# tau-dev/SdfBox

Hardware: AMD Instinct MI355X
Metric: Mray/s (primary rays; frame W*H / time per frame) (higher is better)
Workload: dtype f32

## Files before the change

sdfbox_amd/csrc/raymarch_device.h:

```cpp
#pragma once
#include <hip/hip_runtime.h>
#include <stdint.h>

namespace sdfhip {

typedef uint4 NodeRec;


struct FrameInfo {
    float h0x, h0y, h0z, h1x, h1y, h1z, h2x, h2y, h2z;
    float posx, posy, posz, margin;
    float screen_w, screen_h, limit;
    float lightx, lighty, lightz;
    float fov, k_strength;
    float margin2;
    float half_aspect;
};
constexpr int MAX_BATCH = 8;
constexpr int MAX_BAND_LIST = 512;
constexpr int INLINE_BAND_LIST = 64;

struct TopCell { uint32_t level, v0, v1; int32_t children; };
struct GridRef {
    const TopCell *top; const TopCell *fine; int level; int fine_bits; int fine_order;
#ifdef SDFHIP_EXPERIMENTS
    const uint32_t *d4 = nullptr; const uint4 *recs = nullptr;
    uint32_t *touch_top = nullptr, *touch_fine = nullptr; uint32_t touch_top_words = 0, touch_fine_words = 0;
#endif
};
#ifdef SDFHIP_EXPERIMENTS
__device__ __forceinline__ void touch_line(uint32_t *bits, uint32_t words, uint32_t cell)
// ... 33 lines not shown
    uint32_t n_band_list;
    uint16_t band_list[INLINE_BAND_LIST];
    const uint16_t *band_ptr;
    uint32_t tiles_x, tiles_y, n_tiles;
    uint32_t n_frames;
    FrameInfo frames[MAX_BATCH];
    unsigned long long *counters;
    uint32_t *queue;
#ifdef SDFHIP_EXPERIMENTS
    uint32_t tile_order;
#endif
    uint32_t out_mode;
    uint32_t sparse_cap;
    uint32_t sparse_base;
    uint32_t sky8;
    uint32_t out_host;
    uint32_t pt_spp, pt_bounces, pt_seed;
    float pt_albedo;
    float4 *hit_a;
    int4 *hit_b;
    uint4 *hit_c;
    float4 *hit_d;
    uint32_t *hit_ctl;
    uint32_t hit_cap, hit_set;
    uint32_t hit_min;
    float4 *pt_q[2];
    uint32_t *pt_ctl;
    uint32_t pt_cap, pt_level;
    float *pt_e;
    float *pt_t;
// ... 147 lines not shown
        ax = ay = az = 0; level = 0;
        children = (int32_t)root.y; v0 = root.z; v1 = root.w;
    }
    __device__ __forceinline__ Cell cell() const
    {
        Cell k;
        const float q = 1.0f / 4096.0f;
        k.lx = (float)ax * q; k.ly = (float)ay * q; k.lz = (float)az * q;
        k.scale = __int_as_float((127 - level) << 23);
        k.inv = __int_as_float((127 + level) << 23);
        k.v0 = v0; k.v1 = v1;
        return k;
    }
};

__device__ __forceinline__ int32_t axis_a(float p, float &u, float &f)
{
    u = p * 4096.0f;
    f = floorf(u);
    return (int32_t)__builtin_amdgcn_fmed3f(f, -2.0f, 4097.0f);
}
__device__ __forceinline__ int bitlen(uint32_t x) { return 32 - __clz((int)x); }

template <bool ON_GRID>
__device__ __forceinline__ uint32_t find_s(CursorS &c, const NodeRec *__restrict__ nodes,
                                           const TopCell *__restrict__ top, const int TG,
                                           int32_t *__restrict__ stack, uint32_t stride,
                                           int32_t Ax, int32_t Ay, int32_t Az, bool gx, bool gy, bool gz)
{
    const int32_t Bx = Ax - ((ON_GRID && gx) ? 1 : 0);
    const int32_t By = Ay - ((ON_GRID && gy) ? 1 : 0);
    const int32_t Bz = Az - ((ON_GRID && gz) ? 1 : 0);
    const int s = LM - c.level;
// ... 43 lines not shown
            c.v1 = r.w;
            asm volatile("" : "+v"(c.v0), "+v"(c.v1));
            c.level++;
            reads++; c.loads++;
        }
        const int32_t keep = ~((1 << (LM - c.level)) - 1);
        c.ax = Dx & keep; c.ay = Dy & keep; c.az = Dz & keep;
    } else if (k > 0) {
        const int32_t keep = ~((1 << (LM - c.level)) - 1);
        c.ax &= keep; c.ay &= keep; c.az &= keep;
    }
    return reads;
}

constexpr uint32_t FLAT_BIT = 0x80000000u;
template <bool EXACT, bool SPLIT, bool ORDERED = false>
struct CursorFT {
    typedef Scaled Pos;
    static constexpr int32_t ROOT_MARK = 0x40000000;
    int32_t ax, ay, az;
    uint32_t s;
    uint32_t v0, v1;
    uint32_t sh;
    uint32_t loads;

    __device__ __forceinline__ void reset(const NodeRec &root)
    {
        ax = ay = az = ROOT_MARK; s = (uint32_t)LM; v0 = root.z; v1 = root.w; sh = 0;
    }
    __device__ __forceinline__ int4 pack() const
    {
        const bool fresh = ax == ROOT_MARK;
        return make_int4(fresh ? ax : (int32_t)((uint32_t)ax << sh), fresh ? ay : (int32_t)((uint32_t)ay << sh), fresh ? az : (int32_t)((uint32_t)az << sh), (int32_t)s);
// ... 7 lines not shown
    __device__ __forceinline__ static uint32_t units_shift(int full_level) { return EXACT ? 0u : (uint32_t)(LM - full_level); }
    __device__ __forceinline__ Cell cell() const
    {
        Cell k;
        const float q = 1.0f / 4096.0f;
        const bool fresh = ax == ROOT_MARK;
        const int32_t keep = (int32_t)(0xFFFFFFFFu << (s & 31u));
        const int32_t x = (int32_t)((uint32_t)ax << sh) & keep, y = (int32_t)((uint32_t)ay << sh) & keep, z = (int32_t)((uint32_t)az << sh) & keep;
        k.lx = fresh ? 0.0f : (float)x * q; k.ly = fresh ? 0.0f : (float)y * q; k.lz = fresh ? 0.0f : (float)z * q;
        const uint32_t sc = s & 15u;
        k.scale = __uint_as_float((127u - LM + sc) << 23);
        k.inv = __uint_as_float((127u + LM - sc) << 23);
        k.v0 = v0; k.v1 = (s & FLAT_BIT) ? v0 : v1;
        return k;
    }
};

template <bool EXACT, bool SPLIT, bool ORDERED>
__device__ __forceinline__ int load_cell(CursorFT<EXACT, SPLIT, ORDERED> &c, const GridRef &g, int32_t Dx, int32_t Dy, int32_t Dz)
{
    const int TG = g.level, sh = LM - TG;
    const uint32_t ti = top_index((uint32_t)Dx >> sh, (uint32_t)Dy >> sh, (uint32_t)Dz >> sh, TG);
    uint4 e = reinterpret_cast<const uint4 *>(g.top)[ti];
    c.loads++;
#ifdef SDFHIP_EXPERIMENTS
    if (EXACT && g.touch_top) touch_line(g.touch_top, g.touch_top_words, ti);
#endif
    if (SPLIT) {
        asm volatile("" : "+v"(e.y), "+v"(e.z), "+v"(e.w));
        if (e.x == 15u) {
// ... 2 lines not shown
            const uint32_t m = (1u << FB) - 1u;
            const uint32_t local = fine_cell_index(((uint32_t)Dx >> sh2) & m, ((uint32_t)Dy >> sh2) & m, ((uint32_t)Dz >> sh2) & m, FB, ORDERED ? g.fine_order : 0);
#ifdef SDFHIP_EXPERIMENTS
            if (EXACT && g.touch_fine) touch_line(g.touch_fine, g.touch_fine_words, e.w + local);
#endif
            e = reinterpret_cast<const uint4 *>(g.fine)[e.w + local];
        }
    }
    c.s = e.x;
    c.v0 = e.y;
    c.v1 = e.z;
    c.ax = Dx; c.ay = Dy; c.az = Dz;
    return (int)(e.x & 15u);
}

template <bool SPLIT, bool ORDERED>
__device__ __forceinline__ void load_cell_units(CursorFT<false, SPLIT, ORDERED> &c, const GridRef &g, int32_t Dx, int32_t Dy, int32_t Dz)
{
    uint4 e;
    c.loads++;
    if (!SPLIT) {
        e = reinterpret_cast<const uint4 *>(g.top)[top_index((uint32_t)Dx, (uint32_t)Dy, (uint32_t)Dz, g.level)];
    } else {
        const int FB = g.fine_bits;
        e = reinterpret_cast<const uint4 *>(g.top)[top_index((uint32_t)Dx >> FB, (uint32_t)Dy >> FB, (uint32_t)Dz >> FB, g.level)];
        asm volatile("" : "+v"(e.y), "+v"(e.z), "+v"(e.w));
        if (e.x == 15u) {
            c.loads++;
            const uint32_t m = (1u << FB) - 1u;
            const uint32_t local = fine_cell_index((uint32_t)Dx & m, (uint32_t)Dy & m, (uint32_t)Dz & m, FB, ORDERED ? g.fine_order : 0);
            e = reinterpret_cast<const uint4 *>(g.fine)[e.w + local];
            asm volatile("" : "+v"(e.y), "+v"(e.z), "+v"(e.w));
// ... 40 lines not shown
    }
    uint32_t reads = 1u;
    if (moved) {
        Dx = min(max(Dx, 0), 4095); Dy = min(max(Dy, 0), 4095); Dz = min(max(Dz, 0), 4095);
        const int ns = load_cell(c, g, Dx, Dy, Dz);
        reads = 1u + (uint32_t)k + (uint32_t)((LM - ns) - (level - k));
    }
    return reads;
}
__device__ __forceinline__ int32_t cvt_floor(float u)
{
    int32_t a;
    asm("v_cvt_flr_i32_f32_e32 %0, %1" : "=v"(a) : "v"(u));
    return a;
}
template <bool SPLIT, bool FRESH, bool ORDERED>
__device__ __forceinline__ uint32_t find_units(CursorFT<false, SPLIT, ORDERED> &c, const GridRef &g, float px, float py, float pz, Scaled &u)
{
    const int F = g.level + (SPLIT ? g.fine_bits : 0), sh = LM - F;
    const float unit = __uint_as_float((uint32_t)(127 + F) << 23), top = unit - 1.0f;
    u.x = px * unit; u.y = py * unit; u.z = pz * unit;
    const float fx = __builtin_amdgcn_fractf(u.x), fy = __builtin_amdgcn_fractf(u.y), fz = __builtin_amdgcn_fractf(u.z);
    const float fm = __builtin_fminf(__builtin_fminf(fx, fy), fz);
    int32_t Dx, Dy, Dz;
    if (FRESH || __builtin_expect(__ballot(fm == 0.0f) == 0ull, 1)) {
        Dx = cvt_floor(__builtin_amdgcn_fmed3f(u.x, 0.0f, top)); Dy = cvt_floor(__builtin_amdgcn_fmed3f(u.y, 0.0f, top));
        Dz = cvt_floor(__builtin_amdgcn_fmed3f(u.z, 0.0f, top));
    } else {
        float tx, ty, tz, qx, qy, qz;
        Dx = axis_a(px, tx, qx); Dy = axis_a(py, ty, qy); Dz = axis_a(pz, tz, qz);
        const int4 k = c.pack();
        bool moved;
        on_face_choice(k.x, k.y, k.z, (int)(c.s & 15u), Dx, Dy, Dz, tx == qx, ty == qy, tz == qz, moved);
        Dx = min(max(Dx, 0), 4095) >> sh; Dy = min(max(Dy, 0), 4095) >> sh; Dz = min(max(Dz, 0), 4095) >> sh;
    }
    c.sh = (uint32_t)sh;
    load_cell_units(c, g, Dx, Dy, Dz);
    return 0;
}
template <bool SPLIT, bool ORDERED>
__device__ __forceinline__ uint32_t find(CursorFT<false, SPLIT, ORDERED> &c, const NodeRec *__restrict__, const GridRef &g,
                                         uint32_t, int32_t *__restrict__, uint32_t, float px, float py, float pz,
                                         Scaled &u)
{
    return find_units<SPLIT, false, ORDERED>(c, g, px, py, pz, u);
}
template <class CursorT, class Pos>
__device__ __forceinline__ uint32_t find_fresh(CursorT &c, const NodeRec *__restrict__ nodes, const GridRef &g, uint32_t n,
                                               int32_t *__restrict__ stack, uint32_t stride, float px, float py, float pz, Pos &u)
{
    return find(c, nodes, g, n, stack, stride, px, py, pz, u);
}
template <bool SPLIT, bool ORDERED>
__device__ __forceinline__ uint32_t find_fresh(CursorFT<false, SPLIT, ORDERED> &c, const NodeRec *__restrict__, const GridRef &g,
                                               uint32_t, int32_t *__restrict__, uint32_t, float px, float py, float pz,
                                               Scaled &u)
{
    return find_units<SPLIT, true, ORDERED>(c, g, px, py, pz, u);
}
template <bool SPLIT, bool ORDERED>
__device__ __forceinline__ uint32_t find(CursorFT<true, SPLIT, ORDERED> &c, const NodeRec *__restrict__, const GridRef &g,
                                         uint32_t, int32_t *__restrict__, uint32_t, float px, float py, float pz,
                                         Scaled &u)
{
    float fx, fy, fz;
    const int32_t Ax = axis_a(px, u.x, fx), Ay = axis_a(py, u.y, fy), Az = axis_a(pz, u.z, fz);
    const bool gx = u.x == fx, gy = u.y == fy, gz = u.z == fz;
    return find_full(c, g, Ax, Ay, Az, gx, gy, gz, __ballot(gx || gy || gz) != 0ull);
}
template <bool EXACT, bool SPLIT, bool ORDERED>
__device__ __forceinline__ float sample_after_find(const CursorFT<EXACT, SPLIT, ORDERED> &c, const Scaled &u, float, float, float)
{
    if (c.s & FLAT_BIT) return __uint_as_float(c.v1);
    const float scale = __uint_as_float((c.s + (uint32_t)(127 - LM)) << 23);
    const uint32_t k = c.s - c.sh;
    const float inv = __uint_as_float((127u - k) << 23);
    const int32_t keep = (int32_t)(0xFFFFFFFFu << (k & 31u));
    float dx = sat((u.x - (float)(c.ax & keep)) * inv);
    float dy = sat((u.y - (float)(c.ay & keep)) * inv);
    float dz = sat((u.z - (float)(c.az & keep)) * inv);
    Texels t = decode(c.v0, c.v1);
    float loadL = bilerp(t.v[0], t.v[1], t.v[2], t.v[3], dx, dy);
    float loadH = bilerp(t.v[4], t.v[5], t.v[6], t.v[7], dx, dy);
    return (lerp(loadL, loadH, dz) - 0.25f) * scale * 2.0f;
}
__device__ __forceinline__ uint32_t flat_cell_distance_bits(uint32_t byte, uint32_t s)
{
    const float scale = __uint_as_float((s + (uint32_t)(127 - LM)) << 23);
    return __float_as_uint((unorm8((float)byte) - 0.25f) * scale * 2.0f);
}
// ... 114 lines not shown
```

sdfbox_amd/csrc/raymarch_kernels.h:

```cpp
#pragma once
#include "raymarch_device.h"

namespace sdfhip {

constexpr int MAX_STACK = LM;
#ifndef COMPACT_WAVES_PER_SIMD
#define COMPACT_WAVES_PER_SIMD 8
#endif
#ifndef PATH_WAVES_PER_SIMD
#define PATH_WAVES_PER_SIMD 7
#endif
#ifndef PLAIN_WAVES_PER_SIMD
#define PLAIN_WAVES_PER_SIMD 8
#endif

enum { CUR_GENERIC = 0, CUR_STACK = 1, CUR_STACK_FULL = 2, CUR_STACK_SPLIT = 3, CUR_DENSE4 = 4 };
template <int CUR, bool COUNT> struct CursorOf { typedef CursorG type; };
template <bool COUNT> struct CursorOf<CUR_STACK, COUNT> { typedef CursorS type; };
template <bool COUNT> struct CursorOf<CUR_STACK_FULL, COUNT> { typedef CursorFT<COUNT, false> type; };
template <bool COUNT> struct CursorOf<CUR_STACK_SPLIT, COUNT> { typedef CursorFT<COUNT, true> type; };
__device__ __forceinline__ GridRef grid_of(const RenderParams &P, const TopCell *top = nullptr)
{
#ifdef SDFHIP_EXPERIMENTS
    return GridRef{top ? top : P.top, P.fine, P.top_level, P.fine_bits, P.fine_order, P.d4, P.recs,
                   P.touch_top, P.touch_fine, P.touch_top_words, P.touch_fine_words};
#else
    return GridRef{top ? top : P.top, P.fine, P.top_level, P.fine_bits, P.fine_order};
#endif
}
template <class CursorT>
__device__ __forceinline__ Cell cell_of(const CursorT &c, const RenderParams &) { return c.cell(); }
#ifdef SDFHIP_EXPERIMENTS
template <> struct CursorOf<CUR_DENSE4, false> { typedef CursorFF type; };
__device__ __forceinline__ Cell cell_of(const CursorFF &c, const RenderParams &P) { return cell_of(c, grid_of(P), P.nodes); }
#endif
template <int CUR, bool COUNT> struct ScatterCursorOf { typedef typename CursorOf<CUR, COUNT>::type type; };
template <bool COUNT> struct ScatterCursorOf<CUR_STACK_SPLIT, COUNT> { typedef CursorFT<COUNT, true, true> type; };

enum { PH_PRIMARY = 0, PH_SHADOW = 1, PH_SHADE = 2, PH_IDLE = 3, PH_DONE = 4 };

struct RayState {
    float px, py, pz;
    float dx, dy, dz;
    float prox, angle, dist;
    int n, base, phase;
};
// ... 2 lines not shown
{
    if (!P.n_band_list && P.band_first == 0u && P.band_stride == 1u) return yl;
    const uint32_t band = P.band_shift < 32u ? yl >> P.band_shift : yl / P.band_rows, within = yl - band * P.band_rows;
    if (P.n_band_list) {
        if (band >= P.n_band_list) return 0xFFFFFFFFu;
        const uint32_t b = P.n_band_list <= (uint32_t)INLINE_BAND_LIST ? P.band_list[band] : P.band_ptr[band];
        return b * P.band_rows + within;
    }
    return (P.band_first + band * P.band_stride) * P.band_rows + within;
}

template <class CursorT>
__device__ __forceinline__ void start_pixel(const FrameInfo &I, const NodeRec &root, uint32_t x,
                                            uint32_t y, RayState &r, CursorT &c)
{
    r.px = I.posx; r.py = I.posy; r.pz = I.posz;
    ray(I, x, y, r.dx, r.dy, r.dz);
    r.prox = 1.0f;
    r.angle = 0.0f; r.dist = 0.0f;
    r.n = 0; r.base = 0; r.phase = PH_PRIMARY;
    c.reset(root);
}


__device__ __forceinline__ uint32_t to_unorm8(float c) { return (uint32_t)(sat(c) * 255.0f + 0.5f); }
__device__ __forceinline__ uint32_t gamma8(float c) { return to_unorm8(powf(c, 1.0f / 2.2f)); }
__device__ __forceinline__ uint32_t alpha8(float steps) { return steps >= 1.0f ? 0xFF000000u : 0u; }
__device__ __forceinline__ uint32_t heat8(float steps)
{
    uint32_t q = to_unorm8(steps / 140.0f);
    return q | (q << 8) | (q << 16);
}
__device__ __forceinline__ uint32_t display8(const float4 &v, uint32_t mode)
// ... 117 lines not shown
        if (s == 2) return true;
        if (shade(I, r, c, dst)) return true;
    }
    return check_shadow(I, r, c, dst);
}

template <class CursorT, bool FRESH = false>
__device__ __forceinline__ uint32_t march_step(const RenderParams &P, const FrameInfo &I, RayState &r, CursorT &c,
                                               int32_t *stack, uint32_t stride, const TopCell *top = nullptr)
{
    typename CursorT::Pos u;
    const GridRef g = grid_of(P, top);
    uint32_t reads = FRESH ? find_fresh(c, P.nodes, g, P.n_nodes, stack, stride, r.px, r.py, r.pz, u)
                           : find(c, P.nodes, g, P.n_nodes, stack, stride, r.px, r.py, r.pz, u);
    r.prox = sample_after_find(c, u, r.px, r.py, r.pz);
    float step = r.phase ? r.prox + I.margin : r.prox;
    r.px = __builtin_fmaf(r.dx, step, r.px);
    r.py = __builtin_fmaf(r.dy, step, r.py);
    r.pz = __builtin_fmaf(r.dz, step, r.pz);
    r.n++;
    return reads;
}

#ifndef SDFHIP_EXPERIMENTS
struct StepClasses {};
template <class CursorT>
__device__ __forceinline__ void classify_step(StepClasses &, const CursorT &, const RenderParams &, float, float, float) {}
__device__ __forceinline__ void flush_classes(const RenderParams &, StepClasses &) {}
#else
struct StepClasses { unsigned long long n[6] = {0, 0, 0, 0, 0, 0}; };
template <class CursorT>
// ... 210 lines not shown
{
    const uint32_t xcd = (bid + frame * (P.tiles_y & 7u)) & 7u, j = bid >> 3;
    const uint32_t r = j / P.tiles_x, cx = j - r * P.tiles_x;
    const uint32_t row = r * 8 + xcd;
    return row < P.tiles_y ? row * P.tiles_x + cx : 0xFFFFFFFFu;
}
__device__ __forceinline__ uint32_t *hit_count(const RenderParams &P, uint32_t set, uint32_t f, uint32_t q)
{
    return P.hit_ctl + (((size_t)set * MAX_BATCH + f) * HIT_QUEUES + q) * 32u;
}

template <bool COUNT, class CursorT>
__device__ __forceinline__ bool shadow_march(const RenderParams &P, const FrameInfo &I, RayState &r, CursorT &c,
                                             unsigned long long &cn, unsigned long long &cs, StepClasses *classes = nullptr)
{
    auto header = [&]() { return r.n < 40 && r.prox > -I.margin; };
    auto at_light = [&]() {
        const float lo = __builtin_fminf(__builtin_fminf(r.px, r.py), r.pz), hi = __builtin_fmaxf(__builtin_fmaxf(r.px, r.py), r.pz);
        return r.prox > r.dist || lo < 0.0f || hi > 1.0f;
    };
    for (;;) {
        bool go = ((int)header() & (int)!at_light()) != 0;
        if (go && r.prox < I.margin) {
            float gx, gy, gz;
            gradient(cell_of(c, P), r.px, r.py, r.pz, gx, gy, gz);
            go = !(dot3(gx, gy, gz, r.dx, r.dy, r.dz) < 0.0f);
        }
        if (!go) break;
        const float qx = r.px, qy = r.py, qz = r.pz;
        uint32_t reads = march_step(P, I, r, c, nullptr, 0);
        if (COUNT) { cn += reads; cs += 1; if (classes) classify_step(*classes, c, P, qx, qy, qz); }
    }
    asm volatile("" : "+v"(r.prox), "+v"(r.n));
    return header() && at_light();
}

template <int CUR, bool COUNT, int MODE, bool QUEUE = false>
__global__ __launch_bounds__(64, PLAIN_WAVES_PER_SIMD) void k_march(RenderParams P)
{
    typedef typename CursorOf<CUR, COUNT>::type CursorT;
    const uint32_t f = blockIdx.y;
    FrameInfo I = P.frames[f];
    asm volatile("" : "+s"(I.margin2), "+s"(I.limit));
    {
        const uint32_t a0 = P.width, a1 = P.height, a2 = P.nrows_out, a3 = P.tiles_x, a4 = P.tiles_y, a5 = P.n_band_list, a6 = P.band_first,
                       a7 = P.band_stride, a8 = P.n_tiles;
        const int32_t b0 = P.top_level, b1 = P.fine_bits;
        const void *p0 = P.nodes, *p1 = P.top, *p2 = P.fine, *p3 = P.out, *p4 = P.tile_perm, *p5 = P.tile_cost;
        asm volatile("" :: "s"(a0), "s"(a1), "s"(a2), "s"(a3), "s"(a4), "s"(a5), "s"(a6), "s"(a7), "s"(a8), "s"(b0), "s"(b1),
                     "s"(p0), "s"(p1), "s"(p2), "s"(p3), "s"(p4), "s"(p5));
    }
    uint32_t tile, tx, ty;
    if (P.tile_perm) {
        const uint32_t wg = blockIdx.z * gridDim.x + blockIdx.x;
        const uint32_t e = P.tile_perm[(wg & 7u) * P.perm_per_label + (wg >> 3)];
        tx = e & 0xFFFFu; ty = e >> 16;
        if (ty >= P.tiles_y || tx >= P.tiles_x) return;
        tile = ty * P.tiles_x + tx;
// ... 4 lines not shown
        tile = ty * P.tiles_x + tx;
    }
    const uint32_t lane = threadIdx.x;
    const uint32_t x = tx * 8 + (lane & 7u), yl = ty * 8 + (lane >> 3);
    unsigned long long cn = 0, cs = 0, ct = 0;
    StepClasses classes;
    SparseLane wire_px{0.0f, 0u};
    bool live = x < P.width && yl < P.nrows_out;
    uint32_t y = 0;
    if (live) { y = global_row(P, yl); live = y < P.height; }
    RayState r;
    CursorT c;
    c.loads = 0;
    const NodeRec root = P.nodes[0];
    start_pixel(I, root, live ? x : 0u, live ? y : 0u, r, c);
    auto marching = [&]() { return (r.prox > I.margin2 || r.prox < 0.0f) && r.n < 100; };
    if (live) {
        auto go_on = [&]() { return ((int)marching() & (int)!(dot3(r.px, r.py, r.pz, r.px, r.py, r.pz) > I.limit)) != 0; };
        if (go_on()) {
            float qx = r.px, qy = r.py, qz = r.pz;
            uint32_t reads = march_step<CursorT, true>(P, I, r, c, nullptr, 0);
            if (COUNT) { cn += reads; cs += 1; classify_step(classes, c, P, qx, qy, qz); }
            while (go_on()) {
                if (COUNT) { qx = r.px; qy = r.py; qz = r.pz; }
                reads = march_step(P, I, r, c, nullptr, 0);
                if (COUNT) { cn += reads; cs += 1; classify_step(classes, c, P, qx, qy, qz); }
            }
        }
    }
    asm volatile("" : "+v"(r.prox), "+v"(r.n));
    const int end = !live ? 3 : marching() ? 2 : 1;
    if (P.tile_cost) {
        int m = live ? r.n : 0;
        for (int o = 32; o > 0; o >>= 1) m = max(m, __shfl_xor(m, o));
        if (lane == 0) P.tile_cost[(size_t)f * P.n_tiles + tile] = (uint16_t)m;
    }
    const size_t lidx = (size_t)yl * P.width + x;
    if (end == 2) {
        const PixelSink<MODE> dst(P, f, &wire_px);
        dst.sky(lidx, (float)r.n);
        if (COUNT) ct = (unsigned long long)r.n;
    }
    bool shadow = false;
    if (__ballot(end == 1)) {
        if (end == 1) {
            float lx = I.lightx - r.px, ly = I.lighty - r.py, lz = I.lightz - r.pz;
            const float rl = 1.0f / sqrtf(dot3(lx, ly, lz, lx, ly, lz));
            r.dx = lx * rl; r.dy = ly * rl; r.dz = lz * rl;
            r.px = __builtin_fmaf(r.dx, I.margin, r.px);
            r.py = __builtin_fmaf(r.dy, I.margin, r.py);
            r.pz = __builtin_fmaf(r.dz, I.margin, r.pz);
            float gx, gy, gz;
            gradient(cell_of(c, P), r.px, r.py, r.pz, gx, gy, gz);
            const float rg = 1.0f / sqrtf(dot3(gx, gy, gz, gx, gy, gz));
            r.angle = dot3(r.dx, r.dy, r.dz, gx * rg, gy * rg, gz * rg);
            if (r.angle < 0.0f) {
                const PixelSink<MODE> dst(P, f, &wire_px);
                dst.black(lidx, (float)r.n);
                if (COUNT) ct = (unsigned long long)r.n;
            } else {
                shadow = true;
            }
        }
    }
    bool in_place = !QUEUE;
    if constexpr (QUEUE) in_place = (uint32_t)__popcll(__ballot(shadow)) >= P.hit_min;
    if (in_place) {
        if (shadow) {
            const PixelSink<MODE> dst(P, f, &wire_px);
            const float lx = I.lightx - r.px, ly = I.lighty - r.py, lz = I.lightz - r.pz;
            r.dist = sqrtf(dot3(lx, ly, lz, lx, ly, lz)) / 2.0f;
            r.base = r.n; r.n = 0; r.phase = PH_SHADOW;
            const bool lit = shadow_march<COUNT>(P, I, r, c, cn, cs, &classes);
            if (lit) dst.grey(lidx, r.angle / (r.dist * r.dist) * I.k_strength, (float)(r.base + r.n));
            else dst.black(lidx, (float)(r.base + r.n));
            if (COUNT) ct = (unsigned long long)(r.base + r.n);
        }
        if (P.tile_cost) {
            int m = shadow ? r.n : 0;
            for (int o = 32; o > 0; o >>= 1) m = max(m, __shfl_xor(m, o));
            if (lane == 0) P.tile_cost[(size_t)f * P.n_tiles + tile] |= (uint16_t)(m << 8);
        }
        if (MODE == OUT_SPARSE) sparse2_flush(P, f, tile, lane, wire_px);
        if (COUNT) { flush_counters(P, cn, cs, ct, shadow ? 1u : 0u, c.loads, 0u); flush_classes(P, classes); }
        return;
    }
    if constexpr (QUEUE) {
    const unsigned long long hits = __ballot(shadow);
    if (hits) {
        const uint32_t q = (blockIdx.z * gridDim.x + blockIdx.x) & (HIT_QUEUES - 1u);
        uint32_t base = 0;
        if (lane == 0) base = atomicAdd(hit_count(P, P.hit_set, f, q), (uint32_t)__popcll(hits));
        base = (uint32_t)__builtin_amdgcn_readfirstlane((int)base);
        const uint32_t rank = __builtin_amdgcn_mbcnt_hi((uint32_t)(hits >> 32), __builtin_amdgcn_mbcnt_lo((uint32_t)hits, 0u));
        if (shadow && base + rank < P.hit_cap) {
            const size_t slot = ((size_t)f * HIT_QUEUES + q) * P.hit_cap + base + rank;
            P.hit_a[slot] = make_float4(r.px, r.py, r.pz, r.prox);
            P.hit_b[slot] = c.pack();
            P.hit_c[slot] = make_uint4((uint32_t)lidx, (uint32_t)r.n, c.v0, c.v1);
            P.hit_d[slot] = make_float4(r.dx, r.dy, r.dz, r.angle);
        }
    }
    if (COUNT) flush_counters(P, cn, cs, ct, shadow ? 1u : 0u, c.loads, shadow ? 1u : 0u);
    }
}

template <int CUR, bool COUNT, int MODE>
__global__ __launch_bounds__(64, PLAIN_WAVES_PER_SIMD) void k_shadow(RenderParams P)
{
    typedef typename CursorOf<CUR, COUNT>::type CursorT;
    const uint32_t f = blockIdx.y, lane = threadIdx.x;
    FrameInfo I = P.frames[f];
    asm volatile("" : "+s"(I.margin));
    const PixelSink<MODE> dst(P, f);
    const uint32_t fill = min(*hit_count(P, P.hit_set, f, lane), P.hit_cap);
    if (blockIdx.x == 0 && f == 0)
        for (uint32_t ff = 0; ff < (uint32_t)MAX_BATCH; ff++) *hit_count(P, P.hit_set ^ 1u, ff, lane) = 0u;
    const uint32_t chunks = (fill + 63u) >> 6;
    uint32_t incl = chunks;
    for (int o = 1; o < 64; o <<= 1) { const uint32_t v = __shfl_up(incl, o); if ((int)lane >= o) incl += v; }
    const uint32_t total = (uint32_t)__builtin_amdgcn_readlane((int)incl, 63);
    unsigned long long cn = 0, cs = 0, ct = 0, cl = 0;
    for (uint32_t t = blockIdx.x; t < total; t += gridDim.x) {
        const uint32_t q = (uint32_t)__popcll(__ballot(incl <= t));
        const uint32_t q_incl = (uint32_t)__builtin_amdgcn_readlane((int)incl, (int)q), q_chunks = (uint32_t)__builtin_amdgcn_readlane((int)chunks, (int)q);
        const uint32_t q_fill = (uint32_t)__builtin_amdgcn_readlane((int)fill, (int)q);
        const uint32_t i = (t - (q_incl - q_chunks)) * 64u + lane;
        if (i < q_fill) {
            const size_t slot = ((size_t)f * HIT_QUEUES + q) * P.hit_cap + i;
            const float4 a = P.hit_a[slot], d = P.hit_d[slot];
            const int4 b = P.hit_b[slot];
            const uint4 e = P.hit_c[slot];
            RayState r;
            CursorT c;
            r.px = a.x; r.py = a.y; r.pz = a.z; r.prox = a.w; r.dx = d.x; r.dy = d.y; r.dz = d.z; r.angle = d.w;
            r.base = (int)e.y; r.n = 0; r.phase = PH_SHADOW;
            c.unpack(b, CursorT::units_shift(P.top_level + (CUR == CUR_STACK_SPLIT ? P.fine_bits : 0)));
            c.v0 = e.z; c.v1 = e.w; c.loads = 0;
            const size_t lidx = e.x;
            const float lx = I.lightx - r.px, ly = I.lighty - r.py, lz = I.lightz - r.pz;
            r.dist = sqrtf(dot3(lx, ly, lz, lx, ly, lz)) / 2.0f;
            const bool lit = shadow_march<COUNT>(P, I, r, c, cn, cs);
            if (lit) dst.grey(lidx, r.angle / (r.dist * r.dist) * I.k_strength, (float)(r.base + r.n));
            else dst.black(lidx, (float)(r.base + r.n));
            if (COUNT) { ct += (unsigned long long)(r.base + r.n); cl += c.loads; }
        }
    }
    if (COUNT) flush_counters(P, cn, cs, ct, 0, cl);
}

constexpr int REFILL_MIN = 12;
constexpr int SHADE_MIN = 8;

template <int CUR, bool COUNT>
__global__ __launch_bounds__(64, COMPACT_WAVES_PER_SIMD) void k_compact(RenderParams P)
{
    __shared__ int32_t stack_lds[CUR ? MAX_STACK * 64 : 1];
    __shared__ float4 out_lds[64];
// ... 799 lines not shown
```

sdfbox_amd/csrc/render.hip:

```cpp
#include "raymarch_kernels.h"
#include "tile_order_kernels.h"
#include "scene.h"
#include "abi_guard.h"
#ifdef SDFHIP_EXPERIMENTS
#include "../../include/sdfhip_experimental.h"
#endif

#include <chrono>
#include <cmath>
#include <cstdlib>
#include <cstring>
#include <vector>

using namespace sdfhip;

namespace {

struct Plan {
    bool use_stack = false, compact = false, count = false, grid_lookup = false;
    bool persistent = false;
    int cur = CUR_GENERIC;
    uint32_t out_mode = 0;
    dim3 grid;
    sdfhip_scene::Scratch *sc = nullptr;
// ... 1 lines not shown

void unpack_info(const sdfhip_info *in, FrameInfo &I)
{
    I.h0x = in->heading[0][0]; I.h0y = in->heading[0][1]; I.h0z = in->heading[0][2];
    I.h1x = in->heading[1][0]; I.h1y = in->heading[1][1]; I.h1z = in->heading[1][2];
    I.h2x = in->heading[2][0]; I.h2y = in->heading[2][1]; I.h2z = in->heading[2][2];
    I.posx = in->position[0]; I.posy = in->position[1]; I.posz = in->position[2];
    I.margin = in->margin;
    I.margin2 = in->margin * 2.0f;
    I.screen_w = in->screen_size[0]; I.screen_h = in->screen_size[1];
    I.limit = in->limit;
    I.lightx = in->light[0]; I.lighty = in->light[1]; I.lightz = in->light[2];
    I.fov = in->fov;
    I.k_strength = exp2f(in->strength) - 1.0f;
    I.half_aspect = in->screen_size[0] / in->screen_size[1] * 0.5f;
}

uint32_t sky_through_the_display_pass()
{
    auto q = [](float c) { float v = powf(c, 1.0f / 2.2f); v = v > 1.0f ? 1.0f : (v > 0.0f ? v : 0.0f); return (uint32_t)(v * 255.0f + 0.5f); };
    return q(0.005f) | (q(0.01f) << 8) | (q(0.2f) << 16);
}

int fill_params(sdfhip_scene *s, const RenderCall &c, RenderParams &P, Plan &plan)
{
    if (c.n_frames == 0 || c.n_frames > (uint32_t)MAX_BATCH)
        return fail(SDFHIP_ERR_ARG, "render: n_frames %u outside 1..%d", c.n_frames, MAX_BATCH);
    if (c.width == 0 || c.height == 0 || c.nrows_out == 0 || c.band_rows == 0 || c.band_stride == 0)
        return fail(SDFHIP_ERR_ARG, "render: zero-sized frame or band");
    if ((uint64_t)c.width * c.nrows_out > 0x7FFFFFFFull)
// ... 61 lines not shown
    }
    P.tiles_x = (c.width + 7u) / 8u;
    P.tiles_y = (c.nrows_out + 7u) / 8u;
    P.n_tiles = P.tiles_x * P.tiles_y;
    P.n_frames = c.n_frames;
    for (uint32_t f = 0; f < c.n_frames; f++) unpack_info(c.info + f, P.frames[f]);
    P.out_mode = plan.out_mode;
    P.sparse_cap = c.sparse_cap;
    P.sparse_base = c.sparse_base;
    P.sky8 = sky_through_the_display_pass();
    P.pt_spp = c.pt ? c.pt->spp : 0; P.pt_bounces = c.pt ? c.pt->max_bounces : 0; P.pt_seed = c.pt ? c.pt->seed : 0;
    P.pt_albedo = c.pt ? c.pt->albedo : 0.0f;
    plan.cur = !plan.use_stack ? CUR_GENERIC : (s->d_top && s->fine_bits) ? CUR_STACK_SPLIT :
               (s->d_top && (uint32_t)s->top_level >= s->depth) ? CUR_STACK_FULL : CUR_STACK;
    plan.grid_lookup = plan.cur == CUR_STACK_FULL || plan.cur == CUR_STACK_SPLIT;
    plan.grid = dim3(8u * ((P.tiles_y + 7u) / 8u) * P.tiles_x, c.n_frames);
    if (plan.compact && (!plan.grid_lookup || plan.persistent) && (c.width > 65535u || c.nrows_out > 65535u))
        return fail(SDFHIP_ERR_ARG, "render: the persistent-wave compact kernel packs a pixel's x and row into 16 bits each (frame %u x %u)", c.width, c.nrows_out);
    if (c.sparse && !plan.grid_lookup)
        return fail(SDFHIP_ERR_ARG, "render_sparse: this scene has no full-depth grid (trees deeper than 12 levels or with inconsistent links render dense shares)");
    return SDFHIP_OK;
}

int need_scratch(sdfhip_scene *s, const RenderCall &c, Plan &plan)
{
    if (plan.sc) return SDFHIP_OK;
    return get_scratch(s, c.st, 0, &plan.sc);
}

template <int CUR, bool COUNT>
void launch_march(uint32_t mode, dim3 flat, hipStream_t st, const RenderParams &P)
{
    const dim3 grid = march_grid(P, flat);
    if (!COUNT && P.out_host && mode <= (uint32_t)OUT_HEAT8) {
        if (mode == OUT_RGBA32F)     hipLaunchKernelGGL((k_march<CUR, false, OUT_RGBA32F | OUT_HOST, false>), grid, dim3(64), 0, st, P);
        else if (mode == OUT_GAMMA8) hipLaunchKernelGGL((k_march<CUR, false, OUT_GAMMA8 | OUT_HOST, false>), grid, dim3(64), 0, st, P);
        else                         hipLaunchKernelGGL((k_march<CUR, false, OUT_HEAT8 | OUT_HOST, false>), grid, dim3(64), 0, st, P);
        return;
    }
    if (mode == OUT_RGBA32F)     hipLaunchKernelGGL((k_march<CUR, COUNT, OUT_RGBA32F, false>), grid, dim3(64), 0, st, P);
    else if (mode == OUT_GAMMA8) hipLaunchKernelGGL((k_march<CUR, COUNT, OUT_GAMMA8, false>), grid, dim3(64), 0, st, P);
    else if (mode == OUT_HEAT8)  hipLaunchKernelGGL((k_march<CUR, COUNT, OUT_HEAT8, false>), grid, dim3(64), 0, st, P);
    else                         hipLaunchKernelGGL((k_march<CUR, COUNT, OUT_SPARSE, false>), grid, dim3(64), 0, st, P);
}

int launch_default(sdfhip_scene *s, const RenderCall &c, RenderParams &P, Plan &plan)
{
    hipStream_t st = c.st;
// ... 130 lines not shown
    }
#endif
    P.pt_q[0] = reinterpret_cast<float4 *>(sc->pt_buf);
    P.pt_q[1] = reinterpret_cast<float4 *>(sc->pt_buf + qbytes);
    P.pt_e = reinterpret_cast<float *>(sc->pt_buf + 2 * qbytes);
    P.pt_t = reinterpret_cast<float *>(sc->pt_buf + 2 * qbytes + ebytes);
    P.pt_n = reinterpret_cast<uint32_t *>(sc->pt_buf + 2 * qbytes + ebytes + tbytes);
    P.pt_ctl = sc->ctl + sdfhip_scene::CTL_HIT_WORDS + sdfhip_scene::CTL_QUEUE_WORDS;
    if (plan.cur == CUR_STACK_SPLIT) return plan.count ? launch_pt_pipeline<CUR_STACK_SPLIT, true>(s, grid, st, P) : launch_pt_pipeline<CUR_STACK_SPLIT, false>(s, grid, st, P);
    return plan.count ? launch_pt_pipeline<CUR_STACK_FULL, true>(s, grid, st, P) : launch_pt_pipeline<CUR_STACK_FULL, false>(s, grid, st, P);
}

template <int CUR, bool COUNT>
void launch_queued(uint32_t mode, dim3 grid, dim3 shade_grid, hipStream_t st, const RenderParams &P)
{
    auto go = [&](auto march, auto shade) {
        hipLaunchKernelGGL(march, march_grid(P, grid), dim3(64), 0, st, P);
        hipLaunchKernelGGL(shade, shade_grid, dim3(64), 0, st, P);
    };
    if (mode == OUT_RGBA32F)     go(k_march<CUR, COUNT, OUT_RGBA32F, true>, k_shadow<CUR, COUNT, OUT_RGBA32F>);
    else if (mode == OUT_GAMMA8) go(k_march<CUR, COUNT, OUT_GAMMA8, true>, k_shadow<CUR, COUNT, OUT_GAMMA8>);
    else                         go(k_march<CUR, COUNT, OUT_HEAT8, true>, k_shadow<CUR, COUNT, OUT_HEAT8>);
}

int launch_compact(sdfhip_scene *s, const RenderCall &c, RenderParams &P, Plan &plan)
{
    dim3 shade_grid;
    int rc = prepare_shadow_queue(s, c, P, plan.grid, COMPACT_MIN_LANES, &plan.sc, &shade_grid);
    if (rc != SDFHIP_OK) return rc;
    const uint32_t mode = plan.out_mode;
// ... 432 lines not shown
```

Baseline: 22700.

## March rays in grid-cell units to drop per-step position scaling

Adds grid-unit cursor variants that keep ray positions, margins and limits pre-scaled by 2^level, so the lookup skips the per-step multiply into cell units. Frame constants are precomputed on the host, and positions are converted back to world space at the hit and for the shadow pass. The change touches cursor cell/sample functions, the march and shadow kernels, and launch dispatch. It risks floating-point differences at cell faces and more template instantiations.

```diff
diff --git a/sdfbox_amd/csrc/raymarch_device.h b/sdfbox_amd/csrc/raymarch_device.h
--- a/sdfbox_amd/csrc/raymarch_device.h
+++ b/sdfbox_amd/csrc/raymarch_device.h
@@ -15,6 +15,9 @@
     float fov, k_strength;
     float margin2;
     float half_aspect;
+    float g_unit = 0.0f, g_inv = 0.0f;
+    float g_posx = 0.0f, g_posy = 0.0f, g_posz = 0.0f;
+    float g_margin = 0.0f, g_margin2 = 0.0f, g_limit = 0.0f;
 };
 constexpr int MAX_BATCH = 8;
 constexpr int MAX_BAND_LIST = 512;
@@ -78,6 +81,7 @@
     uint32_t sparse_cap;
     uint32_t sparse_base;
     uint32_t sky8;
+    uint32_t grid_units;
     uint32_t out_host;
     uint32_t pt_spp, pt_bounces, pt_seed;
     float pt_albedo;
@@ -255,9 +259,9 @@
     }
 };
 
-__device__ __forceinline__ int32_t axis_a(float p, float &u, float &f)
-{
-    u = p * 4096.0f;
+__device__ __forceinline__ int32_t axis_a(float p, float &u, float &f, float to_lm = 4096.0f)
+{
+    u = p * to_lm;
     f = floorf(u);
     return (int32_t)__builtin_amdgcn_fmed3f(f, -2.0f, 4097.0f);
 }
@@ -331,9 +335,10 @@
 }
 
 constexpr uint32_t FLAT_BIT = 0x80000000u;
-template <bool EXACT, bool SPLIT, bool ORDERED = false>
+template <bool EXACT, bool SPLIT, bool ORDERED = false, bool GRIDPOS = false>
 struct CursorFT {
     typedef Scaled Pos;
+    static_assert(!(EXACT && GRIDPOS), "the counting cursors work in units of 2^-LM and take world positions");
     static constexpr int32_t ROOT_MARK = 0x40000000;
     int32_t ax, ay, az;
     uint32_t s;
@@ -371,6 +376,18 @@
         k.v0 = v0; k.v1 = (s & FLAT_BIT) ? v0 : v1;
         return k;
     }
+    __device__ __forceinline__ Cell cell_units(float inv_unit) const
+    {
+        Cell k;
+        const bool fresh = ax == ROOT_MARK;
+        const uint32_t sc = s & 15u, ks = sc - sh;
+        const int32_t keep = (int32_t)(0xFFFFFFFFu << (ks & 31u));
+        k.lx = fresh ? 0.0f : (float)(ax & keep); k.ly = fresh ? 0.0f : (float)(ay & keep); k.lz = fresh ? 0.0f : (float)(az & keep);
+        k.scale = __uint_as_float((127u + ks) << 23);
+        k.inv = fresh ? inv_unit : __uint_as_float((127u - ks) << 23);
+        k.v0 = v0; k.v1 = (s & FLAT_BIT) ? v0 : v1;
+        return k;
+    }
 };
 
 template <bool EXACT, bool SPLIT, bool ORDERED>
@@ -403,8 +420,8 @@
     return (int)(e.x & 15u);
 }
 
-template <bool SPLIT, bool ORDERED>
-__device__ __forceinline__ void load_cell_units(CursorFT<false, SPLIT, ORDERED> &c, const GridRef &g, int32_t Dx, int32_t Dy, int32_t Dz)
+template <bool SPLIT, bool ORDERED, bool GP>
+__device__ __forceinline__ void load_cell_units(CursorFT<false, SPLIT, ORDERED, GP> &c, const GridRef &g, int32_t Dx, int32_t Dy, int32_t Dz)
 {
     uint4 e;
     c.loads++;
@@ -475,12 +492,13 @@
     asm("v_cvt_flr_i32_f32_e32 %0, %1" : "=v"(a) : "v"(u));
     return a;
 }
-template <bool SPLIT, bool FRESH, bool ORDERED>
-__device__ __forceinline__ uint32_t find_units(CursorFT<false, SPLIT, ORDERED> &c, const GridRef &g, float px, float py, float pz, Scaled &u)
+template <bool SPLIT, bool FRESH, bool ORDERED, bool GP>
+__device__ __forceinline__ uint32_t find_units(CursorFT<false, SPLIT, ORDERED, GP> &c, const GridRef &g, float px, float py, float pz, Scaled &u)
 {
     const int F = g.level + (SPLIT ? g.fine_bits : 0), sh = LM - F;
     const float unit = __uint_as_float((uint32_t)(127 + F) << 23), top = unit - 1.0f;
-    u.x = px * unit; u.y = py * unit; u.z = pz * unit;
+    if (GP) { u.x = px; u.y = py; u.z = pz; }
+    else { u.x = px * unit; u.y = py * unit; u.z = pz * unit; }
     const float fx = __builtin_amdgcn_fractf(u.x), fy = __builtin_amdgcn_fractf(u.y), fz = __builtin_amdgcn_fractf(u.z);
     const float fm = __builtin_fminf(__builtin_fminf(fx, fy), fz);
     int32_t Dx, Dy, Dz;
@@ -489,7 +507,8 @@
         Dz = cvt_floor(__builtin_amdgcn_fmed3f(u.z, 0.0f, top));
     } else {
         float tx, ty, tz, qx, qy, qz;
-        Dx = axis_a(px, tx, qx); Dy = axis_a(py, ty, qy); Dz = axis_a(pz, tz, qz);
+        const float to_lm = GP ? __uint_as_float((uint32_t)(127 + sh) << 23) : 4096.0f;
+        Dx = axis_a(px, tx, qx, to_lm); Dy = axis_a(py, ty, qy, to_lm); Dz = axis_a(pz, tz, qz, to_lm);
         const int4 k = c.pack();
         bool moved;
         on_face_choice(k.x, k.y, k.z, (int)(c.s & 15u), Dx, Dy, Dz, tx == qx, ty == qy, tz == qz, moved);
@@ -499,12 +518,12 @@
     load_cell_units(c, g, Dx, Dy, Dz);
     return 0;
 }
-template <bool SPLIT, bool ORDERED>
-__device__ __forceinline__ uint32_t find(CursorFT<false, SPLIT, ORDERED> &c, const NodeRec *__restrict__, const GridRef &g,
+template <bool SPLIT, bool ORDERED, bool GP>
+__device__ __forceinline__ uint32_t find(CursorFT<false, SPLIT, ORDERED, GP> &c, const NodeRec *__restrict__, const GridRef &g,
                                          uint32_t, int32_t *__restrict__, uint32_t, float px, float py, float pz,
                                          Scaled &u)
 {
-    return find_units<SPLIT, false, ORDERED>(c, g, px, py, pz, u);
+    return find_units<SPLIT, false, ORDERED, GP>(c, g, px, py, pz, u);
 }
 template <class CursorT, class Pos>
 __device__ __forceinline__ uint32_t find_fresh(CursorT &c, const NodeRec *__restrict__ nodes, const GridRef &g, uint32_t n,
@@ -512,12 +531,12 @@
 {
     return find(c, nodes, g, n, stack, stride, px, py, pz, u);
 }
-template <bool SPLIT, bool ORDERED>
-__device__ __forceinline__ uint32_t find_fresh(CursorFT<false, SPLIT, ORDERED> &c, const NodeRec *__restrict__, const GridRef &g,
+template <bool SPLIT, bool ORDERED, bool GP>
+__device__ __forceinline__ uint32_t find_fresh(CursorFT<false, SPLIT, ORDERED, GP> &c, const NodeRec *__restrict__, const GridRef &g,
                                                uint32_t, int32_t *__restrict__, uint32_t, float px, float py, float pz,
                                                Scaled &u)
 {
-    return find_units<SPLIT, true, ORDERED>(c, g, px, py, pz, u);
+    return find_units<SPLIT, true, ORDERED, GP>(c, g, px, py, pz, u);
 }
 template <bool SPLIT, bool ORDERED>
 __device__ __forceinline__ uint32_t find(CursorFT<true, SPLIT, ORDERED> &c, const NodeRec *__restrict__, const GridRef &g,
@@ -529,12 +548,12 @@
     const bool gx = u.x == fx, gy = u.y == fy, gz = u.z == fz;
     return find_full(c, g, Ax, Ay, Az, gx, gy, gz, __ballot(gx || gy || gz) != 0ull);
 }
-template <bool EXACT, bool SPLIT, bool ORDERED>
-__device__ __forceinline__ float sample_after_find(const CursorFT<EXACT, SPLIT, ORDERED> &c, const Scaled &u, float, float, float)
-{
-    if (c.s & FLAT_BIT) return __uint_as_float(c.v1);
-    const float scale = __uint_as_float((c.s + (uint32_t)(127 - LM)) << 23);
+template <bool EXACT, bool SPLIT, bool ORDERED, bool GP>
+__device__ __forceinline__ float sample_after_find(const CursorFT<EXACT, SPLIT, ORDERED, GP> &c, const Scaled &u, float, float, float)
+{
+    if (c.s & FLAT_BIT) return GP ? __uint_as_float(c.v1) * __uint_as_float((127u + LM - c.sh) << 23) : __uint_as_float(c.v1);
     const uint32_t k = c.s - c.sh;
+    const float scale = __uint_as_float(((GP ? k : c.s) + (uint32_t)(127 - (GP ? 0 : LM))) << 23);
     const float inv = __uint_as_float((127u - k) << 23);
     const int32_t keep = (int32_t)(0xFFFFFFFFu << (k & 31u));
     float dx = sat((u.x - (float)(c.ax & keep)) * inv);
diff --git a/sdfbox_amd/csrc/raymarch_kernels.h b/sdfbox_amd/csrc/raymarch_kernels.h
--- a/sdfbox_amd/csrc/raymarch_kernels.h
+++ b/sdfbox_amd/csrc/raymarch_kernels.h
@@ -14,11 +14,32 @@
 #define PLAIN_WAVES_PER_SIMD 8
 #endif
 
-enum { CUR_GENERIC = 0, CUR_STACK = 1, CUR_STACK_FULL = 2, CUR_STACK_SPLIT = 3, CUR_DENSE4 = 4 };
+enum { CUR_GENERIC = 0, CUR_STACK = 1, CUR_STACK_FULL = 2, CUR_STACK_SPLIT = 3, CUR_DENSE4 = 4, CUR_GRID_FULL = 5, CUR_GRID_SPLIT = 6 };
+constexpr bool cur_is_split(int cur) { return cur == CUR_STACK_SPLIT || cur == CUR_GRID_SPLIT; }
 template <int CUR, bool COUNT> struct CursorOf { typedef CursorG type; };
 template <bool COUNT> struct CursorOf<CUR_STACK, COUNT> { typedef CursorS type; };
 template <bool COUNT> struct CursorOf<CUR_STACK_FULL, COUNT> { typedef CursorFT<COUNT, false> type; };
 template <bool COUNT> struct CursorOf<CUR_STACK_SPLIT, COUNT> { typedef CursorFT<COUNT, true> type; };
+template <bool COUNT> struct CursorOf<CUR_GRID_FULL, COUNT> { typedef CursorFT<COUNT, false, false, !COUNT> type; };
+template <bool COUNT> struct CursorOf<CUR_GRID_SPLIT, COUNT> { typedef CursorFT<COUNT, true, false, !COUNT> type; };
+template <class CursorT> struct RayUnits {
+    static constexpr bool GRID = false;
+    __device__ __forceinline__ static float margin(const FrameInfo &I) { return I.margin; }
+    __device__ __forceinline__ static float margin2(const FrameInfo &I) { return I.margin2; }
+    __device__ __forceinline__ static float limit(const FrameInfo &I) { return I.limit; }
+    __device__ __forceinline__ static float one(const FrameInfo &) { return 1.0f; }
+    __device__ __forceinline__ static float to_units(const FrameInfo &, float world) { return world; }
+    __device__ __forceinline__ static float to_world(const FrameInfo &, float units) { return units; }
+};
+template <bool SPLIT, bool ORDERED> struct RayUnits<CursorFT<false, SPLIT, ORDERED, true>> {
+    static constexpr bool GRID = true;
+    __device__ __forceinline__ static float margin(const FrameInfo &I) { return I.g_margin; }
+    __device__ __forceinline__ static float margin2(const FrameInfo &I) { return I.g_margin2; }
+    __device__ __forceinline__ static float limit(const FrameInfo &I) { return I.g_limit; }
+    __device__ __forceinline__ static float one(const FrameInfo &I) { return I.g_unit; }
+    __device__ __forceinline__ static float to_units(const FrameInfo &I, float world) { return world * I.g_unit; }
+    __device__ __forceinline__ static float to_world(const FrameInfo &I, float units) { return units * I.g_inv; }
+};
 __device__ __forceinline__ GridRef grid_of(const RenderParams &P, const TopCell *top = nullptr)
 {
 #ifdef SDFHIP_EXPERIMENTS
@@ -30,6 +51,10 @@
 }
 template <class CursorT>
 __device__ __forceinline__ Cell cell_of(const CursorT &c, const RenderParams &) { return c.cell(); }
+template <class CursorT>
+__device__ __forceinline__ Cell ray_cell_of(const CursorT &c, const RenderParams &P, const FrameInfo &) { return cell_of(c, P); }
+template <bool SPLIT, bool ORDERED>
+__device__ __forceinline__ Cell ray_cell_of(const CursorFT<false, SPLIT, ORDERED, true> &c, const RenderParams &, const FrameInfo &I) { return c.cell_units(I.g_inv); }
 #ifdef SDFHIP_EXPERIMENTS
 template <> struct CursorOf<CUR_DENSE4, false> { typedef CursorFF type; };
 __device__ __forceinline__ Cell cell_of(const CursorFF &c, const RenderParams &P) { return cell_of(c, grid_of(P), P.nodes); }
@@ -62,9 +87,10 @@
 __device__ __forceinline__ void start_pixel(const FrameInfo &I, const NodeRec &root, uint32_t x,
                                             uint32_t y, RayState &r, CursorT &c)
 {
-    r.px = I.posx; r.py = I.posy; r.pz = I.posz;
+    typedef RayUnits<CursorT> U;
+    r.px = U::GRID ? I.g_posx : I.posx; r.py = U::GRID ? I.g_posy : I.posy; r.pz = U::GRID ? I.g_posz : I.posz;
     ray(I, x, y, r.dx, r.dy, r.dz);
-    r.prox = 1.0f;
+    r.prox = U::one(I);
     r.angle = 0.0f; r.dist = 0.0f;
     r.n = 0; r.base = 0; r.phase = PH_PRIMARY;
     c.reset(root);
@@ -212,7 +238,7 @@
     uint32_t reads = FRESH ? find_fresh(c, P.nodes, g, P.n_nodes, stack, stride, r.px, r.py, r.pz, u)
                            : find(c, P.nodes, g, P.n_nodes, stack, stride, r.px, r.py, r.pz, u);
     r.prox = sample_after_find(c, u, r.px, r.py, r.pz);
-    float step = r.phase ? r.prox + I.margin : r.prox;
+    float step = r.phase ? r.prox + RayUnits<CursorT>::margin(I) : r.prox;
     r.px = __builtin_fmaf(r.dx, step, r.px);
     r.py = __builtin_fmaf(r.dy, step, r.py);
     r.pz = __builtin_fmaf(r.dz, step, r.pz);
@@ -453,16 +479,18 @@
 __device__ __forceinline__ bool shadow_march(const RenderParams &P, const FrameInfo &I, RayState &r, CursorT &c,
                                              unsigned long long &cn, unsigned long long &cs, StepClasses *classes = nullptr)
 {
-    auto header = [&]() { return r.n < 40 && r.prox > -I.margin; };
+    typedef RayUnits<CursorT> U;
+    const float margin = U::margin(I), one = U::one(I);
+    auto header = [&]() { return r.n < 40 && r.prox > -margin; };
     auto at_light = [&]() {
         const float lo = __builtin_fminf(__builtin_fminf(r.px, r.py), r.pz), hi = __builtin_fmaxf(__builtin_fmaxf(r.px, r.py), r.pz);
-        return r.prox > r.dist || lo < 0.0f || hi > 1.0f;
+        return r.prox > r.dist || lo < 0.0f || hi > one;
     };
     for (;;) {
         bool go = ((int)header() & (int)!at_light()) != 0;
-        if (go && r.prox < I.margin) {
+        if (go && r.prox < margin) {
             float gx, gy, gz;
-            gradient(cell_of(c, P), r.px, r.py, r.pz, gx, gy, gz);
+            gradient(ray_cell_of(c, P, I), r.px, r.py, r.pz, gx, gy, gz);
             go = !(dot3(gx, gy, gz, r.dx, r.dy, r.dz) < 0.0f);
         }
         if (!go) break;
@@ -480,7 +508,9 @@
     typedef typename CursorOf<CUR, COUNT>::type CursorT;
     const uint32_t f = blockIdx.y;
     FrameInfo I = P.frames[f];
-    asm volatile("" : "+s"(I.margin2), "+s"(I.limit));
+    typedef RayUnits<CursorT> U;
+    if (U::GRID) asm volatile("" : "+s"(I.g_margin2), "+s"(I.g_limit));
+    else asm volatile("" : "+s"(I.margin2), "+s"(I.limit));
     {
         const uint32_t a0 = P.width, a1 = P.height, a2 = P.nrows_out, a3 = P.tiles_x, a4 = P.tiles_y, a5 = P.n_band_list, a6 = P.band_first,
                        a7 = P.band_stride, a8 = P.n_tiles;
@@ -515,9 +545,9 @@
     c.loads = 0;
     const NodeRec root = P.nodes[0];
     start_pixel(I, root, live ? x : 0u, live ? y : 0u, r, c);
-    auto marching = [&]() { return (r.prox > I.margin2 || r.prox < 0.0f) && r.n < 100; };
+    auto marching = [&]() { return (r.prox > U::margin2(I) || r.prox < 0.0f) && r.n < 100; };
     if (live) {
-        auto go_on = [&]() { return ((int)marching() & (int)!(dot3(r.px, r.py, r.pz, r.px, r.py, r.pz) > I.limit)) != 0; };
+        auto go_on = [&]() { return ((int)marching() & (int)!(dot3(r.px, r.py, r.pz, r.px, r.py, r.pz) > U::limit(I))) != 0; };
         if (go_on()) {
             float qx = r.px, qy = r.py, qz = r.pz;
             uint32_t reads = march_step<CursorT, true>(P, I, r, c, nullptr, 0);
@@ -545,6 +575,7 @@
     bool shadow = false;
     if (__ballot(end == 1)) {
         if (end == 1) {
+            r.px = U::to_world(I, r.px); r.py = U::to_world(I, r.py); r.pz = U::to_world(I, r.pz);
             float lx = I.lightx - r.px, ly = I.lighty - r.py, lz = I.lightz - r.pz;
             const float rl = 1.0f / sqrtf(dot3(lx, ly, lz, lx, ly, lz));
             r.dx = lx * rl; r.dy = ly * rl; r.dz = lz * rl;
@@ -570,10 +601,12 @@
         if (shadow) {
             const PixelSink<MODE> dst(P, f, &wire_px);
             const float lx = I.lightx - r.px, ly = I.lighty - r.py, lz = I.lightz - r.pz;
-            r.dist = sqrtf(dot3(lx, ly, lz, lx, ly, lz)) / 2.0f;
+            const float dist = sqrtf(dot3(lx, ly, lz, lx, ly, lz)) / 2.0f;
+            r.dist = U::to_units(I, dist);
+            r.px = U::to_units(I, r.px); r.py = U::to_units(I, r.py); r.pz = U::to_units(I, r.pz);
             r.base = r.n; r.n = 0; r.phase = PH_SHADOW;
             const bool lit = shadow_march<COUNT>(P, I, r, c, cn, cs, &classes);
-            if (lit) dst.grey(lidx, r.angle / (r.dist * r.dist) * I.k_strength, (float)(r.base + r.n));
+            if (lit) dst.grey(lidx, r.angle / (dist * dist) * I.k_strength, (float)(r.base + r.n));
             else dst.black(lidx, (float)(r.base + r.n));
             if (COUNT) ct = (unsigned long long)(r.base + r.n);
         }
@@ -596,7 +629,7 @@
         const uint32_t rank = __builtin_amdgcn_mbcnt_hi((uint32_t)(hits >> 32), __builtin_amdgcn_mbcnt_lo((uint32_t)hits, 0u));
         if (shadow && base + rank < P.hit_cap) {
             const size_t slot = ((size_t)f * HIT_QUEUES + q) * P.hit_cap + base + rank;
-            P.hit_a[slot] = make_float4(r.px, r.py, r.pz, r.prox);
+            P.hit_a[slot] = make_float4(r.px, r.py, r.pz, U::to_world(I, r.prox));
             P.hit_b[slot] = c.pack();
             P.hit_c[slot] = make_uint4((uint32_t)lidx, (uint32_t)r.n, c.v0, c.v1);
             P.hit_d[slot] = make_float4(r.dx, r.dy, r.dz, r.angle);
@@ -611,8 +644,10 @@
 {
     typedef typename CursorOf<CUR, COUNT>::type CursorT;
     const uint32_t f = blockIdx.y, lane = threadIdx.x;
+    typedef RayUnits<CursorT> U;
     FrameInfo I = P.frames[f];
-    asm volatile("" : "+s"(I.margin));
+    if (U::GRID) asm volatile("" : "+s"(I.g_margin));
+    else asm volatile("" : "+s"(I.margin));
     const PixelSink<MODE> dst(P, f);
     const uint32_t fill = min(*hit_count(P, P.hit_set, f, lane), P.hit_cap);
     if (blockIdx.x == 0 && f == 0)
@@ -636,13 +671,15 @@
             CursorT c;
             r.px = a.x; r.py = a.y; r.pz = a.z; r.prox = a.w; r.dx = d.x; r.dy = d.y; r.dz = d.z; r.angle = d.w;
             r.base = (int)e.y; r.n = 0; r.phase = PH_SHADOW;
-            c.unpack(b, CursorT::units_shift(P.top_level + (CUR == CUR_STACK_SPLIT ? P.fine_bits : 0)));
+            c.unpack(b, CursorT::units_shift(P.top_level + (cur_is_split(CUR) ? P.fine_bits : 0)));
             c.v0 = e.z; c.v1 = e.w; c.loads = 0;
             const size_t lidx = e.x;
             const float lx = I.lightx - r.px, ly = I.lighty - r.py, lz = I.lightz - r.pz;
-            r.dist = sqrtf(dot3(lx, ly, lz, lx, ly, lz)) / 2.0f;
+            const float dist = sqrtf(dot3(lx, ly, lz, lx, ly, lz)) / 2.0f;
+            r.dist = U::to_units(I, dist); r.prox = U::to_units(I, r.prox);
+            r.px = U::to_units(I, r.px); r.py = U::to_units(I, r.py); r.pz = U::to_units(I, r.pz);
             const bool lit = shadow_march<COUNT>(P, I, r, c, cn, cs);
-            if (lit) dst.grey(lidx, r.angle / (r.dist * r.dist) * I.k_strength, (float)(r.base + r.n));
+            if (lit) dst.grey(lidx, r.angle / (dist * dist) * I.k_strength, (float)(r.base + r.n));
             else dst.black(lidx, (float)(r.base + r.n));
             if (COUNT) { ct += (unsigned long long)(r.base + r.n); cl += c.loads; }
         }
diff --git a/sdfbox_amd/csrc/render.hip b/sdfbox_amd/csrc/render.hip
--- a/sdfbox_amd/csrc/render.hip
+++ b/sdfbox_amd/csrc/render.hip
@@ -39,6 +39,18 @@
     I.fov = in->fov;
     I.k_strength = exp2f(in->strength) - 1.0f;
     I.half_aspect = in->screen_size[0] / in->screen_size[1] * 0.5f;
+}
+
+bool grid_unit_constants(FrameInfo &I, int full_level)
+{
+    auto bounded = [](float v) { return !(fabsf(v) > 0x1p40f); };
+    if (!(bounded(I.posx) && bounded(I.posy) && bounded(I.posz) && bounded(I.margin))) return false;
+    const float unit = ldexpf(1.0f, full_level);
+    I.g_unit = unit; I.g_inv = 1.0f / unit;
+    I.g_posx = I.posx * unit; I.g_posy = I.posy * unit; I.g_posz = I.posz * unit;
+    I.g_margin = I.margin * unit; I.g_margin2 = I.margin2 * unit;
+    I.g_limit = I.limit * unit * unit;
+    return true;
 }
 
 uint32_t sky_through_the_display_pass()
@@ -130,6 +142,11 @@
     plan.cur = !plan.use_stack ? CUR_GENERIC : (s->d_top && s->fine_bits) ? CUR_STACK_SPLIT :
                (s->d_top && (uint32_t)s->top_level >= s->depth) ? CUR_STACK_FULL : CUR_STACK;
     plan.grid_lookup = plan.cur == CUR_STACK_FULL || plan.cur == CUR_STACK_SPLIT;
+    if (plan.grid_lookup && !plan.count && !c.pt) {
+        P.grid_units = 1u;
+        for (uint32_t f = 0; f < c.n_frames; f++)
+            if (!grid_unit_constants(P.frames[f], s->top_level + s->fine_bits)) P.grid_units = 0u;
+    }
     plan.grid = dim3(8u * ((P.tiles_y + 7u) / 8u) * P.tiles_x, c.n_frames);
     if (plan.compact && (!plan.grid_lookup || plan.persistent) && (c.width > 65535u || c.nrows_out > 65535u))
         return fail(SDFHIP_ERR_ARG, "render: the persistent-wave compact kernel packs a pixel's x and row into 16 bits each (frame %u x %u)", c.width, c.nrows_out);
@@ -148,6 +165,9 @@
 void launch_march(uint32_t mode, dim3 flat, hipStream_t st, const RenderParams &P)
 {
     const dim3 grid = march_grid(P, flat);
+    if constexpr (!COUNT && (CUR == CUR_STACK_FULL || CUR == CUR_STACK_SPLIT)) {
+        if (P.grid_units) { launch_march<CUR == CUR_STACK_SPLIT ? CUR_GRID_SPLIT : CUR_GRID_FULL, false>(mode, flat, st, P); return; }
+    }
     if (!COUNT && P.out_host && mode <= (uint32_t)OUT_HEAT8) {
         if (mode == OUT_RGBA32F)     hipLaunchKernelGGL((k_march<CUR, false, OUT_RGBA32F | OUT_HOST, false>), grid, dim3(64), 0, st, P);
         else if (mode == OUT_GAMMA8) hipLaunchKernelGGL((k_march<CUR, false, OUT_GAMMA8 | OUT_HOST, false>), grid, dim3(64), 0, st, P);
@@ -308,6 +328,9 @@
 template <int CUR, bool COUNT>
 void launch_queued(uint32_t mode, dim3 grid, dim3 shade_grid, hipStream_t st, const RenderParams &P)
 {
+    if constexpr (!COUNT && (CUR == CUR_STACK_FULL || CUR == CUR_STACK_SPLIT)) {
+        if (P.grid_units) { launch_queued<CUR == CUR_STACK_SPLIT ? CUR_GRID_SPLIT : CUR_GRID_FULL, false>(mode, grid, shade_grid, st, P); return; }
+    }
     auto go = [&](auto march, auto shade) {
         hipLaunchKernelGGL(march, march_grid(P, grid), dim3(64), 0, st, P);
         hipLaunchKernelGGL(shade, shade_grid, dim3(64), 0, st, P);
```

After: 22890, median of 4. Within noise of the previous version (+0.8%).
